# Lightning-AI/lit-llama

Hardware: NVIDIA H100
Metric: LLaMA-7B gptq.int4 decode tokens/sec (higher is better)
Workload: dtype bf16

## Files before the change

lit-llama_b200/csrc/api.cu:

```cuda
#include <algorithm>
#include <cstdlib>
#include <mutex>
#include <utility>
#include <vector>

#include "b2l_common.cuh"

namespace b2l {

extern void* g_attn_timeline;
int decode_step_persistent(const b2l_decode_args* d, b2l_stream_t stream);
int check_adapter_prefix(const b2l_adapter_prefix* pre, const char* who);
int check_lora(const b2l_lora* lo, int N, int K, const char* who);

static thread_local char g_err[512] = "";

void set_error(const char* fmt, ...) {
  va_list ap;
  va_start(ap, fmt);
  vsnprintf(g_err, sizeof(g_err), fmt, ap);
  va_end(ap);
}

int cuda_fail(cudaError_t e, const char* what) {
  set_error("%s: %s (%s)", what, cudaGetErrorString(e), cudaGetErrorName(e));
  (void)cudaGetLastError();
  return (int)e;
}

int sm_count() {
  static int n[B2L_MAX_DEVICES] = {};
  int dev = 0;
  if (cudaGetDevice(&dev) != cudaSuccess || dev < 0 || dev >= B2L_MAX_DEVICES) return 132;
  if (n[dev] == 0) {
    int v = 0;
    if (cudaDeviceGetAttribute(&v, cudaDevAttrMultiProcessorCount, dev) != cudaSuccess || v <= 0) v = 132;
    n[dev] = v;
  }
  return n[dev];
}

}

using namespace b2l;

extern "C" int b2l_version(void) { return 100; }

extern "C" const char* b2l_last_error(void) { return g_err; }

extern "C" int b2l_device_info(int* sm, int* cc_major, int* cc_minor) {
  int dev = 0;
  B2L_CUDA(cudaGetDevice(&dev));
  int a = 0, b = 0, c = 0;
  B2L_CUDA(cudaDeviceGetAttribute(&a, cudaDevAttrMultiProcessorCount, dev));
  B2L_CUDA(cudaDeviceGetAttribute(&b, cudaDevAttrComputeCapabilityMajor, dev));
  B2L_CUDA(cudaDeviceGetAttribute(&c, cudaDevAttrComputeCapabilityMinor, dev));
  if (sm) *sm = a;
  if (cc_major) *cc_major = b;
  if (cc_minor) *cc_minor = c;
  return 0;
}

struct PfWindow { const void* ptr[B2L_PF_SEGMENTS]; unsigned long long bytes[B2L_PF_SEGMENTS]; };

static size_t prefetch_distance() {
  static const long mb = [] { const char* e = getenv("B2L_PF_MB"); return e ? atol(e) : 0L; }();
  return mb > 0 ? (size_t)mb << 20 : 0;
}

static std::vector<PfWindow> prefetch_windows(const b2l_decode_args* d) {
  std::vector<std::pair<const uint8_t*, size_t>> ops;
  const bool w8 = (d->flags & B2L_F_W8) != 0;
  auto add = [&](const b2l_q4_weight& w) {
    ops.push_back({(const uint8_t*)w.qw_mma, w8 ? b2l_w8_tiled_i8_bytes(w.N, w.K) : b2l_q4_tiled_i8_bytes(w.N, w.K)});
  };
  for (int l = 0; l < d->n_layer; ++l) {
    add(d->layers[l].c_attn); add(d->layers[l].c_proj); add(d->layers[l].c_fc12); add(d->layers[l].mlp_proj);
  }
  add(d->lm_head);
  const size_t n = ops.size(), D = prefetch_distance();
  std::vector<PfWindow> out(n, PfWindow{});
  if (D == 0) return out;
  std::vector<size_t> start(n + 1, 0);
  for (size_t j = 0; j < n; ++j) start[j + 1] = start[j] + ops[j].second;
  for (size_t j = 0; j < n; ++j) {
    size_t lo = std::max(start[j] + D, start[j + 1]), hi = start[j + 1] + D;
    int sg = 0;
    size_t k = j + 1;
    size_t base = start[j + 1];
    while (lo < hi && sg < B2L_PF_SEGMENTS && k < j + 1 + n) {
      const auto& op = ops[k % n];
      const size_t op_lo = base, op_hi = base + op.second;
      if (lo < op_hi) {
        const size_t a = (lo - op_lo) & ~(size_t)127, b = std::min(hi, op_hi) - op_lo;
        if (b > a && op.first != nullptr) {
          out[j].ptr[sg] = op.first + a;
          out[j].bytes[sg] = (b - a + 15) & ~(size_t)15;
          ++sg;
        }
        lo = std::min(hi, op_hi);
      }
      base = op_hi;
      ++k;
    }
  }
  return out;
}

static int q4_call(const b2l_q4_weight& w, const void* x, int ldx, void* y, int ldy, int M, int sz_dtype, int prologue,
                   const void* norm_scale, float eps, int epilogue, const void* res, int ldres, int flags,
                   b2l_stream_t stream, void* trace = nullptr, void* batch_work = nullptr, const PfWindow* pf = nullptr,
                   const b2l_decode_args* kv_of = nullptr, int kv_layer = 0, const b2l_out_affine* aff = nullptr) {
  b2l_q4_linear_args a{};
  if (aff != nullptr) a.out_affine = *aff;
  if (kv_of != nullptr) {
    const int hs = kv_of->n_embd / kv_of->n_head;
    a.pf_kv[0] = kv_of->layers[kv_layer].k_cache; a.pf_kv[1] = kv_of->layers[kv_layer].v_cache;
    a.pf_rows = (const long long*)kv_of->input_pos;
    a.pf_rows_max = kv_of->S; a.pf_nseg = kv_of->B * kv_of->n_head; a.pf_row_bytes = hs * 2;
    a.pf_seg_stride = (unsigned long long)kv_of->S * hs * 2;
  }
  if (pf != nullptr)
    for (int i = 0; i < B2L_PF_SEGMENTS; ++i) { a.pf_ptr[i] = pf->ptr[i]; a.pf_bytes[i] = pf->bytes[i]; }
  a.x = x; a.ldx = ldx;
  const bool gemv = (M == 1 && w.qw_mma != nullptr);
  const bool batch = (!gemv && M <= 8 && w.qw_mma != nullptr && batch_work != nullptr);
  a.qw_tiled = (gemv || batch) ? w.qw_mma : w.qw_tiled; a.scales = w.scales; a.zeros = w.zeros; a.sz_dtype = sz_dtype;
  a.y = y; a.ldy = ldy;
  a.M = M; a.N = w.N; a.K = w.K;
  a.prologue = prologue; a.norm_scale = norm_scale; a.eps = eps;
  a.epilogue = epilogue; a.res = res; a.ldres = ldres;
  a.split_k = 0;
  a.flags = flags;
  a.trace = gemv ? trace : nullptr;
  if ((flags & B2L_F_Q4_BATCH_I8) && M > 1) {
    a.qw_tiled = w.qw_mma; a.trace = nullptr; a.workspace = batch_work;
    a.flags = flags & B2L_F_PDL;
    return b2l_q4_gemv_batch_i8(&a, stream);
  }
  if (flags & B2L_F_W8) {
    if (M > 1) {
      a.qw_tiled = w.qw_mma; a.trace = nullptr; a.workspace = batch_work;
      a.flags = flags & B2L_F_PDL;
      return b2l_w8_gemv_batch(&a, stream);
    }
    a.flags = flags & (B2L_F_PDL | B2L_F_DEBUG_NOCOMPUTE);
    return b2l_w8_gemv(&a, stream);
  }
  if (gemv) return b2l_q4_gemv(&a, stream);
  if (batch) {
    a.workspace = batch_work;
    return b2l_q4_gemv_batch(&a, stream);
  }
  if (a.qw_tiled == nullptr) {
    set_error("b2l_decode_step: weight has no tiling for batch %d", M);
    return B2L_E_STATE;
  }
  return b2l_q4_linear_tc(&a, stream);
}

static int q8_call(const b2l_decode_args* d, const b2l_q8_weight& w, const b2l_q8_weight* w2, const void* x, void* y,
                   const void* norm_scale, int epilogue, const void* res, const b2l_out_affine* aff, b2l_stream_t stream) {
  b2l_q8_linear_args a{};
  a.x = x; a.cb = w.cb; a.scb = w.scb;
  if (w2 != nullptr) { a.cb2 = w2->cb; a.scb2 = w2->scb; }
  a.y = y; a.N = w.N; a.K = w.K; a.threshold = d->q8_threshold;
  a.prologue = norm_scale != nullptr ? B2L_PRO_RMSNORM : B2L_PRO_NONE; a.norm_scale = norm_scale; a.eps = d->eps;
  a.epilogue = epilogue; a.res = res;
  if (aff != nullptr) a.out_affine = *aff;
  a.flags = d->flags & B2L_F_PDL;
  if (d->flags & B2L_F_Q8_BATCH)
    return b2l_q8_linear_batch(&a, d->B, d->batch_work, b2l_q8_linear_batch_workspace_bytes(w.K, d->B), stream);
  return b2l_q8_linear(&a, stream);
}

static int check_q8_weight(const b2l_q8_weight& w, int N, int K, const char* what, int l) {
// ... 85 lines not shown
  if (q8)
    if (int rc = check_q8(d)) return rc;
  if (d->flags & B2L_F_W8_BATCH) {
    B2L_CHECK_SUPPORTED(d->flags & B2L_F_W8, "b2l_decode_step: B2L_F_W8_BATCH needs B2L_F_W8 (gptq.int8)");
    B2L_CHECK_SUPPORTED(d->B >= 2 && d->B <= 16, "b2l_decode_step: B2L_F_W8_BATCH runs batches of 2..16, got B=%d", d->B);
    B2L_CHECK_SUPPORTED(d->plan == nullptr, "b2l_decode_step: B2L_F_W8_BATCH does not run in the persistent kernel (plan must be NULL)");
    B2L_CHECK_SUPPORTED(d->affines == nullptr && d->lm_head_affine.scale == nullptr && d->lm_head_affine.bias == nullptr,
                        "b2l_decode_step: B2L_F_W8_BATCH does not apply LLaMA-Adapter v2 affines (batch 1 only)");
    B2L_CHECK_ARG(d->batch_work != nullptr, "b2l_decode_step: B2L_F_W8_BATCH needs batch_work (b2l_w8_gemv_batch_workspace_bytes(max K, B) bytes)");
  } else if (d->flags & B2L_F_W8) {
    B2L_CHECK_SUPPORTED(d->B == 1, "b2l_decode_step: B2L_F_W8 (gptq.int8) runs batch 1 only, got B=%d", d->B);
    B2L_CHECK_SUPPORTED(d->plan == nullptr, "b2l_decode_step: B2L_F_W8 (gptq.int8) does not run in the persistent kernel (plan must be NULL)");
  }
  if (d->adapters != nullptr) {
    for (int l = 0; l < d->n_layer; ++l) {
      if (d->adapters[l].len == 0) continue;
      B2L_CHECK_SUPPORTED(d->plan == nullptr, "b2l_decode_step: adapters do not run in the persistent kernel (plan must be NULL)");
      if (int rc = check_adapter_prefix(&d->adapters[l], "b2l_decode_step")) return rc;
    }
  }
  if (d->loras != nullptr) {
    for (int l = 0; l < d->n_layer; ++l) {
      if (d->loras[l].r == 0) continue;
      B2L_CHECK_SUPPORTED(d->plan == nullptr, "b2l_decode_step: LoRA layers do not run in the persistent kernel (plan must be NULL)");
      if (int rc = check_lora(&d->loras[l], 3 * d->n_embd, d->n_embd, "b2l_decode_step")) return rc;
    }
  }
  const bool any_affine = d->affines != nullptr || d->lm_head_affine.scale != nullptr || d->lm_head_affine.bias != nullptr;
  if (any_affine) {
    B2L_CHECK_SUPPORTED(d->B == 1 || (d->flags & B2L_F_Q8_BATCH),
                        "b2l_decode_step: LLaMA-Adapter v2 affines run at batch 1 only, got B=%d", d->B);
    B2L_CHECK_SUPPORTED(d->plan == nullptr, "b2l_decode_step: LLaMA-Adapter v2 affines do not run in the persistent kernel (plan must be NULL)");
    B2L_CHECK_SUPPORTED(d->loras == nullptr, "b2l_decode_step: LLaMA-Adapter v2 affines and LoRA do not combine");
    auto ok = [](const b2l_out_affine& f) { return (f.scale == nullptr) == (f.bias == nullptr); };
    B2L_CHECK_ARG(ok(d->lm_head_affine), "b2l_decode_step: lm_head_affine needs both scale and bias (or neither)");
    B2L_CHECK_SUPPORTED(q8 || d->lm_head.qw_mma != nullptr, "b2l_decode_step: affines need the batch-1 tiling (qw_mma) of every weight");
    for (int l = 0; d->affines != nullptr && l < d->n_layer; ++l) {
      const b2l_layer_affine& f = d->affines[l];
      B2L_CHECK_ARG(ok(f.c_attn) && ok(f.c_proj) && ok(f.c_fc12) && ok(f.mlp_proj),
                    "b2l_decode_step: affines[%d] needs both scale and bias (or neither) per linear", l);
      const b2l_layer& L = d->layers[l];
      B2L_CHECK_SUPPORTED(q8 || (L.c_attn.qw_mma && L.c_proj.qw_mma && L.c_fc12.qw_mma && L.mlp_proj.qw_mma),
                          "b2l_decode_step: affines need the batch-1 tiling (qw_mma) of every weight");
    }
  }
  if (d->plan != nullptr) return decode_step_persistent(d, stream);
  const int C = d->n_embd, hs = C / d->n_head, B = d->B;
  const int fl = d->flags & ~(B2L_F_ROW_POS | B2L_F_STEPWISE);
  const int afl = d->flags & ~(B2L_F_W8 | B2L_F_Q8 | B2L_F_W8_BATCH | B2L_F_Q4_BATCH_I8 | B2L_F_Q8_BATCH);
  int rc;
  char* tlb = (char*)d->timeline;
  int li = 0;
  auto tl = [&]() -> void* { void* r = tlb ? (void*)(tlb + 512 * li) : nullptr; ++li; return r; };
  std::vector<PfWindow> pfw;
  if (B == 1 && d->lm_head.qw_mma != nullptr) pfw = prefetch_windows(d);
  static const int kv_prefetch = [] { const char* e = getenv("B2L_KV_PREFETCH"); return e ? atoi(e) : 0; }();
  const bool kv_ok = B == 1 && hs == 128 && d->lm_head.qw_mma != nullptr;
  int oi = 0;
  auto pf = [&]() -> const PfWindow* { const PfWindow* r = pfw.empty() ? nullptr : &pfw[oi]; ++oi; return r; };
  if ((rc = row_pos ? b2l_ring_advance_rows(d->input_pos, B, d->ring_start, d->S, stream)
                    : b2l_ring_advance(d->input_pos, stepwise ? B : 1, d->ring_start, d->S, stream)))
    return rc;
  const int aB = stepwise ? 1 : B, aT = stepwise ? B : 1;
  if ((rc = b2l_embedding(d->idx, d->idx_is_i64, d->wte, d->x, B, C, d->vocab, stream))) return rc;
  for (int l = 0; l < d->n_layer; ++l) {
    const b2l_layer& L = d->layers[l];
    const b2l_layer_affine* af = d->affines != nullptr ? &d->affines[l] : nullptr;
    const b2l_q8_layer* Q = q8 ? &d->q8_layers[l] : nullptr;
    void* t = tl();
    if ((rc = Q ? q8_call(d, Q->c_attn, nullptr, d->x, d->qkv, L.rms_1, B2L_EPI_STORE, nullptr, af ? &af->c_attn : nullptr, stream)
                : q4_call(L.c_attn, d->x, C, d->qkv, 3 * C, B, d->sz_dtype, B2L_PRO_RMSNORM, L.rms_1, d->eps, B2L_EPI_STORE,
                          nullptr, 0, fl, stream, t, d->batch_work, pf(), (kv_ok && kv_prefetch == 2) ? d : nullptr, l,
                          af ? &af->c_attn : nullptr)))
      return rc;
    if (d->loras != nullptr && d->loras[l].r != 0 &&
        (rc = b2l_lora_apply(&d->loras[l], d->x, C, L.rms_1, d->eps, d->qkv, 3 * C, B, 3 * C, C, fl & B2L_F_PDL, stream)))
      return rc;
    g_attn_timeline = tl();
    const b2l_adapter_prefix* pre = (d->adapters != nullptr && d->adapters[l].len != 0) ? &d->adapters[l] : nullptr;
    if ((rc = pre != nullptr
                  ? b2l_attention_adapter(d->qkv, L.k_cache, L.v_cache, d->rope, d->input_pos, d->ring_start, d->att,
                                          d->attn_work, aB, aT, d->n_head, hs, d->S, d->block_size, afl, pre, stream)
                  : b2l_attention(d->qkv, L.k_cache, L.v_cache, d->rope, d->input_pos, d->ring_start, d->att,
                                  d->attn_work, aB, aT, d->n_head, hs, d->S, d->block_size, afl, stream))) {
      g_attn_timeline = nullptr;
      return rc;
    }
    g_attn_timeline = nullptr;
    t = tl();
    if ((rc = Q ? q8_call(d, Q->c_proj, nullptr, d->att, d->x, nullptr, B2L_EPI_RESIDUAL, d->x, af ? &af->c_proj : nullptr, stream)
                : q4_call(L.c_proj, d->att, C, d->x, C, B, d->sz_dtype, B2L_PRO_NONE, nullptr, 0.f, B2L_EPI_RESIDUAL, d->x, C,
                          fl, stream, t, d->batch_work, pf(), nullptr, 0, af ? &af->c_proj : nullptr)))
      return rc;
    t = tl();
    if ((rc = Q ? q8_call(d, Q->c_fc1, &Q->c_fc2, d->x, d->hid, L.rms_2, B2L_EPI_SWIGLU, nullptr, af ? &af->c_fc12 : nullptr, stream)
                : q4_call(L.c_fc12, d->x, C, d->hid, d->n_hidden, B, d->sz_dtype, B2L_PRO_RMSNORM, L.rms_2, d->eps,
                          B2L_EPI_SWIGLU, nullptr, 0, fl, stream, t, d->batch_work, pf(), nullptr, 0, af ? &af->c_fc12 : nullptr)))
      return rc;
    const bool kvpf = kv_prefetch == 1 && kv_ok && l + 1 < d->n_layer;
    t = tl();
    if ((rc = Q ? q8_call(d, Q->mlp_proj, nullptr, d->hid, d->x, nullptr, B2L_EPI_RESIDUAL, d->x, af ? &af->mlp_proj : nullptr, stream)
                : q4_call(L.mlp_proj, d->hid, d->n_hidden, d->x, C, B, d->sz_dtype, B2L_PRO_NONE, nullptr, 0.f,
                          B2L_EPI_RESIDUAL, d->x, C, fl, stream, t, d->batch_work, pf(), kvpf ? d : nullptr, l + 1,
                          af ? &af->mlp_proj : nullptr)))
      return rc;
  }
  if (q8) return q8_call(d, d->q8_lm_head, nullptr, d->x, d->logits, d->ln_f, B2L_EPI_STORE, nullptr, &d->lm_head_affine, stream);
  return q4_call(d->lm_head, d->x, C, d->logits, d->vocab, B, d->sz_dtype, B2L_PRO_RMSNORM, d->ln_f, d->eps,
                 B2L_EPI_STORE, nullptr, 0, fl, stream, tl(), d->batch_work, pf(), nullptr, 0, &d->lm_head_affine);
}
```

lit-llama_b200/csrc/q4_gemv.cu:

```cuda
#include <cstdlib>

#include "q4_mma_common.cuh"

namespace b2l {
namespace q4mv {

struct Params {
  const __nv_bfloat16* x;
  const uint8_t* qwt;
  const void* scales; const void* zeros; int szdt;
  __nv_bfloat16* y;
  int N, K;
  int n_rb;
  int prologue; const __nv_bfloat16* norm_scale; float eps;
  int epilogue; const __nv_bfloat16* res;
  int nst;
  unsigned long long* tl;
  int nocompute;
  const uint8_t* pf_ptr[B2L_PF_SEGMENTS];
  uint32_t pf_bytes[B2L_PF_SEGMENTS];
  int pf_mode;
  const uint8_t* pf_kv[2]; const long long* pf_rows; int pf_rows_max, pf_nseg, pf_row_bytes; unsigned long long pf_seg_stride;
  int evict_first;
  const __nv_bfloat16* aff_scale; const __nv_bfloat16* aff_bias;
};

constexpr uint32_t PF_CHUNK = 16384;

__host__ __device__ inline uint32_t plane_stride(int K) { return (uint32_t)K + ((K % 128 == 0) ? 64u : 0u); }

struct SmemLayout {
  uint32_t ring, xf, zero, scratch, red, sxp, bars, total;
};
__host__ __device__ inline SmemLayout smem_layout(int nst, int K, int ndig) {
  SmemLayout L;
  uint32_t o = 0;
  L.ring = o;    o += (uint32_t)nst * STAGE_BYTES;
  L.xf = o;      o += (uint32_t)ndig * plane_stride(K);
  L.zero = o;    o += 16;
  L.scratch = o; o += 2 * NCW * MAX_HALVES * RB * 16;
  L.red = o;     o += 144;
  L.sxp = o;     o += NCW * 32 * 4;
  L.bars = o;    o += 2 * MAX_STAGES * 8;
  L.total = (o + 127u) & ~127u;
  return L;
}

__device__ __forceinline__ void l2_prefetch_bulk(const void* src, uint32_t bytes) {
  asm volatile("cp.async.bulk.prefetch.L2.global [%0], %1;" ::"l"(src), "r"(bytes) : "memory");
}
__device__ __forceinline__ void l2_prefetch_line(const void* src) {
  asm volatile("prefetch.global.L2 [%0];" ::"l"(src));
}
__device__ __forceinline__ void pf_slice(uint32_t bytes, uint32_t& lo, uint32_t& hi) {
  const uint32_t lines = (bytes + 127u) >> 7;
  lo = (uint32_t)(((unsigned long long)blockIdx.x * lines) / gridDim.x) << 7;
  hi = min((uint32_t)(((unsigned long long)(blockIdx.x + 1) * lines) / gridDim.x) << 7, bytes);
}
__device__ __forceinline__ void tma_bulk_g2s_hint(uint32_t dst, const void* src, uint32_t bytes, uint32_t mbar, uint64_t policy) {
  asm volatile(
      "cp.async.bulk.shared::cluster.global.mbarrier::complete_tx::bytes.L2::cache_hint [%0], [%1], %2, [%3], %4;" ::"r"(dst),
      "l"(src), "r"(bytes), "r"(mbar), "l"(policy)
      : "memory");
}

__device__ __forceinline__ uint32_t balanced_digits(int X) { return ((uint32_t)X + 0x00808080u) ^ 0x00808080u; }

template <bool W8> struct WTile {
  static constexpr int KB_BYTES = W8 ? 1024 : 512;
  static constexpr int KBP = HALF_STAGE_BYTES / KB_BYTES;
};

template <bool W8>
__device__ __forceinline__ void single_imma(int (&a)[2][4], const uint8_t* tile, const uint4& xb) {
  if constexpr (W8) {
    const uint4 w0 = *reinterpret_cast<const uint4*>(tile), w1 = *reinterpret_cast<const uint4*>(tile + 512);
    mma_u8s8_16832(a[0], w0.x, w0.y, w0.z, w0.w, xb.x, xb.y);
    mma_u8s8_16832(a[1], w1.x, w1.y, w1.z, w1.w, xb.z, xb.w);
  } else {
    const uint4 wv = *reinterpret_cast<const uint4*>(tile);
    mma_u8s8_16832(a[0], wv.x, wv.x & 0xf0f0f0f0u, wv.y, wv.y & 0xf0f0f0f0u, xb.x, xb.y);
    mma_u8s8_16832(a[1], wv.z, wv.z & 0xf0f0f0f0u, wv.w, wv.w & 0xf0f0f0f0u, xb.z, xb.w);
  }
}

template <int NH, bool W8>
__device__ __forceinline__ void kblock_imma(int (&acc)[MAX_HALVES][2][4], const uint8_t* wbase, const uint4& xb) {
#pragma unroll
  for (int h = 0; h < NH; ++h) single_imma<W8>(acc[h], wbase + h * HALF_STAGE_BYTES, xb);
}

template <int MAXC, int NDIG, bool W8, bool AFFINE>
__global__ void __launch_bounds__(NTHREADS, 2) q4_gemv_kernel(const Params p) {
  constexpr int KB_BYTES = WTile<W8>::KB_BYTES, KBP_PER_STAGE = WTile<W8>::KBP;
  extern __shared__ __align__(128) uint8_t smem[];
  const SmemLayout L = smem_layout(p.nst, p.K, NDIG);
  const uint32_t sbase = smem_u32(smem);
  const int tid = threadIdx.x, warp = tid >> 5, lane = tid & 31;
  const int n_kb = p.K / KB;
  const int spu2 = (n_kb + KBP_PER_STAGE - 1) / KBP_PER_STAGE, spu1 = (n_kb + 2 * KBP_PER_STAGE - 1) / (2 * KBP_PER_STAGE);
  const int rb_lo = (int)(((long long)blockIdx.x * p.n_rb) / gridDim.x);
  const int rb_hi = (int)(((long long)(blockIdx.x + 1) * p.n_rb) / gridDim.x);
  const int n_units = (rb_hi - rb_lo + 1) / 2;
  const int total_stages = ((rb_hi - rb_lo) / 2) * spu2 + ((rb_hi - rb_lo) & 1) * spu1;
  const uint32_t bar_full = sbase + L.bars, bar_empty = bar_full + MAX_STAGES * 8;
  const uint32_t PS = plane_stride(p.K);

  if (tid == 0) tl_min(p.tl, 0);
  if (tid == 0) {
    for (int i = 0; i < p.nst; ++i) {
      mbar_init(bar_full + i * 8, 1);
      mbar_init(bar_empty + i * 8, NCW);
    }
    asm volatile("fence.mbarrier_init.release.cluster;" ::: "memory");
  }
  if (tid < 4) reinterpret_cast<uint32_t*>(smem + L.zero)[tid] = 0u;
  __syncthreads();

  if (warp == PRODUCER_WARP) {
    if (lane == 0) {
      int slot = 0;
      uint32_t phase = 1;
      int it = 0;
      uint64_t policy = 0;
      if (p.evict_first) asm volatile("createpolicy.fractional.L2::evict_first.b64 %0, 1.0;" : "=l"(policy));
      for (int u = 0; u < n_units; ++u) {
        const int rb = rb_lo + 2 * u;
        const int halves = min(2, rb_hi - rb);
        const uint8_t* src = p.qwt + (size_t)rb * n_kb * KB_BYTES;
        const int per_stage = halves == 2 ? KBP_PER_STAGE : 2 * KBP_PER_STAGE;
        for (int kb0 = 0; kb0 < n_kb; kb0 += per_stage, ++it) {
          const int nkb = min(per_stage, n_kb - kb0);
          const uint32_t bytes = (uint32_t)nkb * KB_BYTES;
          mbar_wait(bar_empty + slot * 8, phase);
          mbar_expect_tx(bar_full + slot * 8, bytes * halves);
          for (int h = 0; h < halves; ++h) {
            const uint32_t dst = sbase + L.ring + slot * STAGE_BYTES + h * HALF_STAGE_BYTES;
            const uint8_t* from = src + ((size_t)h * n_kb + kb0) * KB_BYTES;
            if (p.evict_first) tma_bulk_g2s_hint(dst, from, bytes, bar_full + slot * 8, policy);
            else tma_bulk_g2s(dst, from, bytes, bar_full + slot * 8);
          }
          if (++slot == p.nst) { slot = 0; phase ^= 1; }
          if (it + 1 == min(total_stages, p.nst)) {
            pdl_launch_dependents();
            if (p.pf_mode == 1) {
#pragma unroll
              for (int sgi = 0; sgi < B2L_PF_SEGMENTS; ++sgi) {
                if (p.pf_bytes[sgi] == 0) continue;
                uint32_t lo, hi;
                pf_slice(p.pf_bytes[sgi], lo, hi);
#pragma unroll 1
                for (uint32_t o = lo; o < hi; o += PF_CHUNK) l2_prefetch_bulk(p.pf_ptr[sgi] + o, min(PF_CHUNK, hi - o));
              }
            }
          }
        }
      }
      if (total_stages == 0) pdl_launch_dependents();
      if (p.pf_kv[0] != nullptr) {
        long long rows = *p.pf_rows;
        rows = rows < 0 ? 0 : (rows > p.pf_rows_max ? p.pf_rows_max : rows);
        const uint32_t seg_bytes = (uint32_t)rows * (uint32_t)p.pf_row_bytes;
        const uint32_t cps = (seg_bytes + PF_CHUNK - 1) / PF_CHUNK;
        const uint32_t total = 2u * (uint32_t)p.pf_nseg * cps;
#pragma unroll 1
        for (uint32_t id = blockIdx.x; id < total; id += gridDim.x) {
          const uint32_t sg = id / cps, o = (id - sg * cps) * PF_CHUNK;
          const uint32_t which = sg >= (uint32_t)p.pf_nseg ? 1u : 0u;
          const uint8_t* base = p.pf_kv[which] + (size_t)(sg - which * p.pf_nseg) * p.pf_seg_stride;
          l2_prefetch_bulk(base + o, min(PF_CHUNK, seg_bytes - o));
        }
      }
    }
  } else if (warp < NCW) {
    float* red = reinterpret_cast<float*>(smem + L.red);
    int* red_sh = reinterpret_cast<int*>(smem + L.red + 128);
    {
      const bool norm = (p.prologue == B2L_PRO_RMSNORM);
      constexpr int NT = NCW * 32;
      constexpr uint32_t MAGIC_BITS = 0x4B400000u;
      uint4 xv[MAXC], gv[MAXC];
#pragma unroll
      for (int c = 0; c < MAXC; ++c) {
        const int k = (c * NT + tid) * 8;
        gv[c] = make_uint4(0, 0, 0, 0);
        if (norm && k < p.K) gv[c] = *reinterpret_cast<const uint4*>(p.norm_scale + k);
      }
      pdl_wait();
      if (tid == 0) tl_max(p.tl, 1);
#pragma unroll
      for (int c = 0; c < MAXC; ++c) {
        const int k = (c * NT + tid) * 8;
        xv[c] = make_uint4(0, 0, 0, 0);
        if (k < p.K) xv[c] = ld_coherent_u4(p.x + k);
      }
      const int nchunk = (p.K + NT * 8 - 1) / (NT * 8);
      float ss = 0.f;
      __nv_bfloat162 amax2 = __float2bfloat162_rn(0.f);
#pragma unroll
      for (int c = 0; c < MAXC; ++c) {
        if (c < nchunk) {
          const uint32_t w[4] = {xv[c].x, xv[c].y, xv[c].z, xv[c].w};
          const uint32_t g[4] = {gv[c].x, gv[c].y, gv[c].z, gv[c].w};
#pragma unroll
          for (int q = 0; q < 4; ++q) {
            const __nv_bfloat162 v = *reinterpret_cast<const __nv_bfloat162*>(&w[q]);
            if (norm) {
              amax2 = __hmax2(amax2, __habs2(__hmul2(v, *reinterpret_cast<const __nv_bfloat162*>(&g[q]))));
              const __nv_bfloat162 sq = __hmul2(v, v);
              const uint32_t su = *reinterpret_cast<const uint32_t*>(&sq);
              ss += __uint_as_float(su << 16) + __uint_as_float(su & 0xffff0000u);
            } else {
              amax2 = __hmax2(amax2, __habs2(v));
            }
          }
        }
      }
      float mx = fmaxf(__low2float(amax2), __high2float(amax2));
      ss = warp_sum(ss);
      mx = warp_max(mx);
      if (lane == 0) { red[warp] = ss; red[8 + warp] = mx; }
      named_bar_sync(1, NT);
      ss = 0.f; mx = 0.f;
#pragma unroll
      for (int w = 0; w < NCW; ++w) { ss += red[w]; mx = fmaxf(mx, red[8 + w]); }
// ... 89 lines not shown
              for (int i = 0; i < NPAIR; ++i) {
                const int kbl = i * NCW + warp;
                if (kbl < nkb) kblock_imma<MAX_HALVES, W8>(acc, st_base + kbl * KB_BYTES, *reinterpret_cast<const uint4*>(xq + kbl * xf_step));
              }
            }
          } else {
            if (nkb == 2 * KBP_PER_STAGE) {
#pragma unroll
              for (int i = 0; i < NSINGLE; ++i) {
                const int kbl = i * NCW + warp;
                single_imma<W8>(acc[i & 1], st_base + kbl * KB_BYTES, *reinterpret_cast<const uint4*>(xq + kbl * xf_step));
              }
            } else {
#pragma unroll
              for (int i = 0; i < NSINGLE; ++i) {
                const int kbl = i * NCW + warp;
                if (kbl < nkb) single_imma<W8>(acc[i & 1], st_base + kbl * KB_BYTES, *reinterpret_cast<const uint4*>(xq + kbl * xf_step));
              }
            }
          }
        }
        __syncwarp();
        if (lane == 0) mbar_arrive(bar_empty + slot * 8);
        if (++slot == p.nst) { slot = 0; phase ^= 1; }
      }
      const int buf = u & 1;
      named_bar_sync(4 + buf, NCW * 32 + 32);
      if (t4 < 2) {
        if (halves != MAX_HALVES) {
#pragma unroll
          for (int c = 0; c < 2; ++c)
#pragma unroll
            for (int i = 0; i < 4; ++i) acc[0][c][i] += acc[1][c][i];
        }
#pragma unroll
        for (int h = 0; h < MAX_HALVES; ++h) {
          const int c0 = acc[h][0][0] + acc[h][1][0], c1 = acc[h][0][1] + acc[h][1][1];
          const int c2 = acc[h][0][2] + acc[h][1][2], c3 = acc[h][0][3] + acc[h][1][3];
          int* dst = scratch + (((buf * NCW + warp) * MAX_HALVES + h) * RB + (lane >> 2)) * 4 + 2 * t4;
          if constexpr (W8) {
            *reinterpret_cast<int2*>(dst) = make_int2(c0, c1);
            *reinterpret_cast<int2*>(dst + 8 * 4) = make_int2(c2, c3);
          } else {
            *reinterpret_cast<int2*>(dst) = make_int2(c0 - c2, c1 - c3);
            *reinterpret_cast<int2*>(dst + 8 * 4) = make_int2(c2 >> 4, c3 >> 4);
          }
        }
      }
      __syncwarp();
      named_bar_arrive(6 + buf, NCW * 32 + 32);
    }
    if (tid == 0) tl_max(p.tl, 3);
  } else {
    if (p.pf_mode >= 2) {
      const uint32_t step = p.pf_mode == 2 ? 128u : 32u;
#pragma unroll
      for (int sgi = 0; sgi < B2L_PF_SEGMENTS; ++sgi) {
        if (p.pf_bytes[sgi] == 0) continue;
        uint32_t lo, hi;
        pf_slice(p.pf_bytes[sgi], lo, hi);
#pragma unroll 1
        for (uint32_t o = lo + lane * step; o < hi; o += 32 * step) l2_prefetch_line(p.pf_ptr[sgi] + o);
      }
    }
    float aff_s = 1.f, aff_b = 0.f;
    auto load_affine = [&](int u) {
      const int orow = (rb_lo + 2 * u + (lane >> 4)) * RB + (lane & 15);
      const int o = min(orow, p.N - 1);
      aff_s = bf2f(p.aff_scale[o]);
      aff_b = bf2f(p.aff_bias[o]);
    };
    if constexpr (AFFINE) {
      if (n_units > 0) load_affine(0);
    }
    pdl_wait();
    const int* red_sh = reinterpret_cast<const int*>(smem + L.red + 128);
    const int* scratch = reinterpret_cast<const int*>(smem + L.scratch);
    named_bar_sync(3, NCW * 32 + 32);
    long long sum_x = 0;
    {
      const int4* sp = reinterpret_cast<const int4*>(smem + L.sxp) + lane * 2;
      const int4 s0 = sp[0], s1 = sp[1];
      sum_x = (long long)s0.x + s0.y + s0.z + s0.w + s1.x + s1.y + s1.z + s1.w;
#pragma unroll
      for (int o = 16; o > 0; o >>= 1) sum_x += __shfl_xor_sync(0xffffffffu, sum_x, o);
    }
    const double dsum_x = (double)sum_x;
    const int sh = *red_sh;
    const double inv_scale = __longlong_as_double((long long)(1023 - sh) << 52);
    if (n_units > 0) named_bar_arrive(4, NCW * 32 + 32);
    if (n_units > 1) named_bar_arrive(5, NCW * 32 + 32);
    for (int u = 0; u < n_units; ++u) {
      const int rb = rb_lo + 2 * u;
      const int halves = min(2, rb_hi - rb);
      const int buf = u & 1;
      const int half = lane >> 4, row = lane & 15;
      const bool active = half < halves;
      const int orow = (rb + half) * RB + row;
      const int o = min(orow, p.N - 1);
      const float sc = load_sz(p.scales, p.szdt, o);
      const float zero = load_sz(p.zeros, p.szdt, o);
      if constexpr (AFFINE) {
        if (u > 0) load_affine(u);
      }
      float resv = 0.f;
      if (p.epilogue == B2L_EPI_RESIDUAL && active && orow < p.N) resv = bf2f(p.res[orow]);
      named_bar_sync(6 + buf, NCW * 32 + 32);
      int d0 = 0, d1 = 0, d2 = 0, d3 = 0;
#pragma unroll
      for (int w = 0; w < NCW; ++w) {
        const int4 v = *reinterpret_cast<const int4*>(scratch + (((buf * NCW + w) * MAX_HALVES + half) * RB + row) * 4);
        d0 += v.x; d1 += v.y; d2 += v.z; d3 += v.w;
      }
      if (u + 2 < n_units) named_bar_arrive(4 + buf, NCW * 32 + 32);
      const long long tq = (long long)d0 + ((long long)d1 << 8) + ((long long)d2 << 16) + ((long long)d3 << 24);
      const float tf = (float)(((double)tq - (double)zero * dsum_x) * inv_scale);
      float v = rbf(sc * tf);
// ... 92 lines not shown

using namespace b2l;
using namespace b2l::q4mv;

extern "C" size_t b2l_q4_tiled_i8_bytes(int N, int K) {
  if (N <= 0 || K <= 0 || K % KB != 0) return 0;
  return (size_t)((N + RB - 1) / RB) * (K / KB) * KB_BYTES;
}

extern "C" int b2l_q4_tile_i8(const void* qw, void* qw_tiled, int N, int K, b2l_stream_t stream) {
  B2L_CHECK_ARG(qw && qw_tiled && N > 0 && K > 0, "b2l_q4_tile_i8: bad argument");
  B2L_CHECK_SUPPORTED(K % KB == 0, "b2l_q4_tile_i8: in_features %d must be a multiple of %d", K, KB);
  const size_t total = b2l_q4_tiled_i8_bytes(N, K) / 4;
  q4_tile_i8_kernel<<<(unsigned)((total + 255) / 256), 256, 0, (cudaStream_t)stream>>>((const uint8_t*)qw, (uint32_t*)qw_tiled, N, K);
  B2L_LAUNCH_CHECK("q4_tile_i8_kernel");
  return 0;
}

extern "C" int b2l_q4_untile_i8(const void* qw_tiled, void* qw, int N, int K, b2l_stream_t stream) {
  B2L_CHECK_ARG(qw && qw_tiled && N > 0 && K > 0, "b2l_q4_untile_i8: bad argument");
  B2L_CHECK_SUPPORTED(K % KB == 0, "b2l_q4_untile_i8: in_features %d must be a multiple of %d", K, KB);
  const size_t total = (size_t)(K / 2) * N;
  q4_untile_i8_kernel<<<(unsigned)((total + 255) / 256), 256, 0, (cudaStream_t)stream>>>((const uint32_t*)qw_tiled, (uint8_t*)qw, N, K);
  B2L_LAUNCH_CHECK("q4_untile_i8_kernel");
  return 0;
}

extern "C" size_t b2l_w8_tiled_i8_bytes(int N, int K) {
  if (N <= 0 || K <= 0 || K % KB != 0) return 0;
  return (size_t)((N + RB - 1) / RB) * (K / KB) * WTile<true>::KB_BYTES;
}

extern "C" int b2l_w8_tile_i8(const void* qw, void* qw_tiled, int N, int K, b2l_stream_t stream) {
  B2L_CHECK_ARG(qw && qw_tiled && N > 0 && K > 0, "b2l_w8_tile_i8: bad argument");
  B2L_CHECK_SUPPORTED(K % KB == 0, "b2l_w8_tile_i8: in_features %d must be a multiple of %d", K, KB);
  const size_t total = b2l_w8_tiled_i8_bytes(N, K) / 4;
  w8_tile_i8_kernel<<<(unsigned)((total + 255) / 256), 256, 0, (cudaStream_t)stream>>>((const uint8_t*)qw, (uint32_t*)qw_tiled, N, K);
  B2L_LAUNCH_CHECK("w8_tile_i8_kernel");
  return 0;
}

extern "C" int b2l_w8_untile_i8(const void* qw_tiled, void* qw, int N, int K, b2l_stream_t stream) {
  B2L_CHECK_ARG(qw && qw_tiled && N > 0 && K > 0, "b2l_w8_untile_i8: bad argument");
  B2L_CHECK_SUPPORTED(K % KB == 0, "b2l_w8_untile_i8: in_features %d must be a multiple of %d", K, KB);
  const size_t total = (size_t)K * N;
  w8_untile_i8_kernel<<<(unsigned)((total + 255) / 256), 256, 0, (cudaStream_t)stream>>>((const uint8_t*)qw_tiled, (uint8_t*)qw, N, K);
  B2L_LAUNCH_CHECK("w8_untile_i8_kernel");
  return 0;
}

namespace {
constexpr int MAX_K = 12 * NCW * 32 * 8;

template <int MAXC, int NDIG, bool W8, bool AFFINE>
int launch_gemv_variant(const Params& p0, int ctas_per_sm, int grid_override, bool pdl, cudaStream_t stream) {
  Params p = p0;
  static const int env_kb = [] { const char* e = getenv("B2L_GEMV_SMEM_KB"); return e ? atoi(e) : 0; }();
  const uint32_t budget = (env_kb > 0 ? (uint32_t)env_kb : (ctas_per_sm >= 2 ? 110u : 224u)) * 1024u;
  const uint32_t fixed = smem_layout(0, p.K, NDIG).total;
  int nst = fixed + 2 * STAGE_BYTES <= budget ? (int)((budget - fixed) / STAGE_BYTES) : 0;
  if (nst > MAX_STAGES) nst = MAX_STAGES;
  static const int env_nst = [] { const char* e = getenv("B2L_GEMV_STAGES"); return e ? atoi(e) : 0; }();
  if (env_nst > 0 && nst > env_nst) nst = env_nst;
  if (nst < 2) {
    set_error("b2l_q4_gemv: K=%d does not leave room for the weight ring", p.K);
    return B2L_E_UNSUPPORTED;
  }
  p.nst = nst;
  const SmemLayout L = smem_layout(nst, p.K, NDIG);
  static DynSmemCache smem_cache;
  if (int rc = ensure_dyn_smem(q4_gemv_kernel<MAXC, NDIG, W8, AFFINE>, L.total, smem_cache)) return rc;
  int grid = grid_override > 0 ? grid_override : ctas_per_sm * sm_count();
  if (grid > p.n_rb) grid = p.n_rb;
  LaunchCfg lc(dim3(grid), dim3(NTHREADS), L.total, stream, pdl, 1);
  B2L_CUDA(cudaLaunchKernelEx(&lc.cfg, q4_gemv_kernel<MAXC, NDIG, W8, AFFINE>, p));
  return 0;
}

template <int MAXC, int NDIG, bool W8>
int launch_gemv(const Params& p, int ctas_per_sm, int grid_override, bool pdl, cudaStream_t stream) {
  if (p.aff_scale != nullptr) return launch_gemv_variant<MAXC, NDIG, W8, true>(p, ctas_per_sm, grid_override, pdl, stream);
  return launch_gemv_variant<MAXC, NDIG, W8, false>(p, ctas_per_sm, grid_override, pdl, stream);
}

template <bool W8>
int gemv_entry(const b2l_q4_linear_args* a, b2l_stream_t stream) {
  const char* fn = W8 ? "b2l_w8_gemv" : "b2l_q4_gemv";
  B2L_CHECK_ARG(a != nullptr, "%s: null args", fn);
  B2L_CHECK_ARG(a->x && a->qw_tiled && a->scales && a->zeros && a->y, "%s: null pointer", fn);
  B2L_CHECK_SUPPORTED(a->M == 1, "%s: M=%d (this kernel is the batch-1 path; use %s)", fn, a->M,
                      W8 ? "b2l_w8_gemm" : "b2l_q4_gemv_batch / b2l_q4_linear_tc");
  B2L_CHECK_SUPPORTED(a->K > 0 && a->K % KB == 0 && a->K <= MAX_K, "%s: K=%d must be a multiple of %d and <= %d", fn, a->K, KB, MAX_K);
  B2L_CHECK_ARG(a->N > 0, "%s: bad N", fn);
  B2L_CHECK_ARG(((uintptr_t)a->x % 16 == 0) && ((uintptr_t)a->qw_tiled % 16 == 0), "%s: x / qw_tiled must be 16-byte aligned", fn);
  B2L_CHECK_ARG(a->sz_dtype == B2L_BF16 || a->sz_dtype == B2L_F32, "%s: bad sz_dtype", fn);
  if (W8) B2L_CHECK_SUPPORTED((a->flags & ~(B2L_F_PDL | B2L_F_DEBUG_NOCOMPUTE)) == 0, "%s: unknown flags 0x%x", fn, a->flags);
  if (a->prologue == B2L_PRO_RMSNORM)
    B2L_CHECK_ARG(a->norm_scale && ((uintptr_t)a->norm_scale % 16 == 0), "%s: RMSNorm prologue needs a 16-byte aligned scale", fn);
  else
    B2L_CHECK_ARG(a->prologue == B2L_PRO_NONE, "%s: bad prologue %d", fn, a->prologue);
  if (a->epilogue == B2L_EPI_RESIDUAL) B2L_CHECK_ARG(a->res != nullptr, "%s: RESIDUAL epilogue needs res", fn);
  else if (a->epilogue == B2L_EPI_SWIGLU) B2L_CHECK_SUPPORTED(a->N % RB == 0, "%s: SWIGLU needs N %% 16 == 0", fn);
  else B2L_CHECK_ARG(a->epilogue == B2L_EPI_STORE, "%s: bad epilogue %d", fn, a->epilogue);
  B2L_CHECK_ARG((a->out_affine.scale == nullptr) == (a->out_affine.bias == nullptr),
                "%s: out_affine needs both scale and bias (or neither)", fn);

  Params p;
  p.aff_scale = (const __nv_bfloat16*)a->out_affine.scale;
  p.aff_bias = (const __nv_bfloat16*)a->out_affine.bias;
  p.x = (const __nv_bfloat16*)a->x;
  p.qwt = (const uint8_t*)a->qw_tiled;
  p.scales = a->scales; p.zeros = a->zeros; p.szdt = a->sz_dtype;
  p.y = (__nv_bfloat16*)a->y;
  p.N = a->N; p.K = a->K;
  p.n_rb = (a->N + RB - 1) / RB;
  p.prologue = a->prologue; p.norm_scale = (const __nv_bfloat16*)a->norm_scale; p.eps = a->eps;
  p.epilogue = a->epilogue; p.res = (const __nv_bfloat16*)a->res;
  p.nst = 0;
  p.tl = (unsigned long long*)a->trace;
  p.nocompute = (a->flags & B2L_F_DEBUG_NOCOMPUTE) ? 1 : 0;
  static const int env_pf_mode = [] { const char* e = getenv("B2L_PF_MODE"); return e ? atoi(e) : 1; }();
  static const int env_evict = [] { const char* e = getenv("B2L_PF_EVICT"); return e ? atoi(e) : 0; }();
  p.pf_mode = 0;
  p.evict_first = env_evict;
  p.pf_kv[0] = p.pf_kv[1] = nullptr; p.pf_rows = nullptr; p.pf_rows_max = p.pf_nseg = p.pf_row_bytes = 0; p.pf_seg_stride = 0;
  if (a->pf_kv[0] != nullptr) {
    B2L_CHECK_ARG(a->pf_kv[1] != nullptr && a->pf_rows != nullptr && a->pf_rows_max > 0 && a->pf_nseg > 0 && a->pf_row_bytes > 0 &&
                      a->pf_row_bytes % 16 == 0 && a->pf_seg_stride % 16 == 0 && ((uintptr_t)a->pf_kv[0] % 16 == 0) &&
                      ((uintptr_t)a->pf_kv[1] % 16 == 0) && (unsigned long long)a->pf_rows_max * a->pf_row_bytes < (1ull << 31),
                  "%s: bad strided prefetch hint", fn);
    p.pf_kv[0] = (const uint8_t*)a->pf_kv[0]; p.pf_kv[1] = (const uint8_t*)a->pf_kv[1];
    p.pf_rows = a->pf_rows; p.pf_rows_max = a->pf_rows_max; p.pf_nseg = a->pf_nseg; p.pf_row_bytes = a->pf_row_bytes;
    p.pf_seg_stride = a->pf_seg_stride;
  }
  for (int i = 0; i < B2L_PF_SEGMENTS; ++i) {
    p.pf_ptr[i] = (const uint8_t*)a->pf_ptr[i];
    p.pf_bytes[i] = 0;
    if (a->pf_ptr[i] != nullptr && a->pf_bytes[i] != 0) {
      B2L_CHECK_ARG(((uintptr_t)a->pf_ptr[i] % 16 == 0) && (a->pf_bytes[i] % 16 == 0) && a->pf_bytes[i] < (1ull << 31),
                    "%s: prefetch segment %d must be 16-byte aligned, a multiple of 16 and < 2 GiB", fn, i);
      p.pf_bytes[i] = (uint32_t)a->pf_bytes[i];
      p.pf_mode = env_pf_mode;
    }
  }
  static const int env_cps = [] { const char* e = getenv("B2L_GEMV_CTAS_PER_SM"); return e ? atoi(e) : 0; }();
  const bool pdl = (a->flags & B2L_F_PDL) != 0;
  cudaStream_t st = (cudaStream_t)stream;
  const int grid = a->split_k;
  if (a->K <= 12288) return launch_gemv<6, 3, W8>(p, env_cps > 0 ? env_cps : 2, grid, pdl, st);
  if (a->K <= 16384) return launch_gemv<12, 3, W8>(p, env_cps > 0 ? env_cps : 2, grid, pdl, st);
  return launch_gemv<12, 3, W8>(p, 1, grid, pdl, st);
}
}

extern "C" int b2l_q4_gemv(const b2l_q4_linear_args* a, b2l_stream_t stream) { return gemv_entry<false>(a, stream); }

extern "C" int b2l_w8_gemv(const b2l_q4_linear_args* a, b2l_stream_t stream) { return gemv_entry<true>(a, stream); }
```

Before: 596.3.

## Drop L2 prefetch machinery and pick one CTA per SM when the ring holds all stages

```diff
diff --git a/lit-llama_b200/csrc/api.cu b/lit-llama_b200/csrc/api.cu
--- a/lit-llama_b200/csrc/api.cu
+++ b/lit-llama_b200/csrc/api.cu
@@ -1,8 +1,4 @@
-#include <algorithm>
-#include <cstdlib>
 #include <mutex>
-#include <utility>
-#include <vector>
 
 #include "b2l_common.cuh"
 
@@ -61,67 +57,11 @@
   return 0;
 }
 
-struct PfWindow { const void* ptr[B2L_PF_SEGMENTS]; unsigned long long bytes[B2L_PF_SEGMENTS]; };
-
-static size_t prefetch_distance() {
-  static const long mb = [] { const char* e = getenv("B2L_PF_MB"); return e ? atol(e) : 0L; }();
-  return mb > 0 ? (size_t)mb << 20 : 0;
-}
-
-static std::vector<PfWindow> prefetch_windows(const b2l_decode_args* d) {
-  std::vector<std::pair<const uint8_t*, size_t>> ops;
-  const bool w8 = (d->flags & B2L_F_W8) != 0;
-  auto add = [&](const b2l_q4_weight& w) {
-    ops.push_back({(const uint8_t*)w.qw_mma, w8 ? b2l_w8_tiled_i8_bytes(w.N, w.K) : b2l_q4_tiled_i8_bytes(w.N, w.K)});
-  };
-  for (int l = 0; l < d->n_layer; ++l) {
-    add(d->layers[l].c_attn); add(d->layers[l].c_proj); add(d->layers[l].c_fc12); add(d->layers[l].mlp_proj);
-  }
-  add(d->lm_head);
-  const size_t n = ops.size(), D = prefetch_distance();
-  std::vector<PfWindow> out(n, PfWindow{});
-  if (D == 0) return out;
-  std::vector<size_t> start(n + 1, 0);
-  for (size_t j = 0; j < n; ++j) start[j + 1] = start[j] + ops[j].second;
-  for (size_t j = 0; j < n; ++j) {
-    size_t lo = std::max(start[j] + D, start[j + 1]), hi = start[j + 1] + D;
-    int sg = 0;
-    size_t k = j + 1;
-    size_t base = start[j + 1];
-    while (lo < hi && sg < B2L_PF_SEGMENTS && k < j + 1 + n) {
-      const auto& op = ops[k % n];
-      const size_t op_lo = base, op_hi = base + op.second;
-      if (lo < op_hi) {
-        const size_t a = (lo - op_lo) & ~(size_t)127, b = std::min(hi, op_hi) - op_lo;
-        if (b > a && op.first != nullptr) {
-          out[j].ptr[sg] = op.first + a;
-          out[j].bytes[sg] = (b - a + 15) & ~(size_t)15;
-          ++sg;
-        }
-        lo = std::min(hi, op_hi);
-      }
-      base = op_hi;
-      ++k;
-    }
-  }
-  return out;
-}
-
 static int q4_call(const b2l_q4_weight& w, const void* x, int ldx, void* y, int ldy, int M, int sz_dtype, int prologue,
                    const void* norm_scale, float eps, int epilogue, const void* res, int ldres, int flags,
-                   b2l_stream_t stream, void* trace = nullptr, void* batch_work = nullptr, const PfWindow* pf = nullptr,
-                   const b2l_decode_args* kv_of = nullptr, int kv_layer = 0, const b2l_out_affine* aff = nullptr) {
+                   b2l_stream_t stream, void* trace = nullptr, void* batch_work = nullptr, const b2l_out_affine* aff = nullptr) {
   b2l_q4_linear_args a{};
   if (aff != nullptr) a.out_affine = *aff;
-  if (kv_of != nullptr) {
-    const int hs = kv_of->n_embd / kv_of->n_head;
-    a.pf_kv[0] = kv_of->layers[kv_layer].k_cache; a.pf_kv[1] = kv_of->layers[kv_layer].v_cache;
-    a.pf_rows = (const long long*)kv_of->input_pos;
-    a.pf_rows_max = kv_of->S; a.pf_nseg = kv_of->B * kv_of->n_head; a.pf_row_bytes = hs * 2;
-    a.pf_seg_stride = (unsigned long long)kv_of->S * hs * 2;
-  }
-  if (pf != nullptr)
-    for (int i = 0; i < B2L_PF_SEGMENTS; ++i) { a.pf_ptr[i] = pf->ptr[i]; a.pf_bytes[i] = pf->bytes[i]; }
   a.x = x; a.ldx = ldx;
   const bool gemv = (M == 1 && w.qw_mma != nullptr);
   const bool batch = (!gemv && M <= 8 && w.qw_mma != nullptr && batch_work != nullptr);
@@ -313,12 +253,6 @@
   char* tlb = (char*)d->timeline;
   int li = 0;
   auto tl = [&]() -> void* { void* r = tlb ? (void*)(tlb + 512 * li) : nullptr; ++li; return r; };
-  std::vector<PfWindow> pfw;
-  if (B == 1 && d->lm_head.qw_mma != nullptr) pfw = prefetch_windows(d);
-  static const int kv_prefetch = [] { const char* e = getenv("B2L_KV_PREFETCH"); return e ? atoi(e) : 0; }();
-  const bool kv_ok = B == 1 && hs == 128 && d->lm_head.qw_mma != nullptr;
-  int oi = 0;
-  auto pf = [&]() -> const PfWindow* { const PfWindow* r = pfw.empty() ? nullptr : &pfw[oi]; ++oi; return r; };
   if ((rc = row_pos ? b2l_ring_advance_rows(d->input_pos, B, d->ring_start, d->S, stream)
                     : b2l_ring_advance(d->input_pos, stepwise ? B : 1, d->ring_start, d->S, stream)))
     return rc;
@@ -331,8 +265,7 @@
     void* t = tl();
     if ((rc = Q ? q8_call(d, Q->c_attn, nullptr, d->x, d->qkv, L.rms_1, B2L_EPI_STORE, nullptr, af ? &af->c_attn : nullptr, stream)
                 : q4_call(L.c_attn, d->x, C, d->qkv, 3 * C, B, d->sz_dtype, B2L_PRO_RMSNORM, L.rms_1, d->eps, B2L_EPI_STORE,
-                          nullptr, 0, fl, stream, t, d->batch_work, pf(), (kv_ok && kv_prefetch == 2) ? d : nullptr, l,
-                          af ? &af->c_attn : nullptr)))
+                          nullptr, 0, fl, stream, t, d->batch_work, af ? &af->c_attn : nullptr)))
       return rc;
     if (d->loras != nullptr && d->loras[l].r != 0 &&
         (rc = b2l_lora_apply(&d->loras[l], d->x, C, L.rms_1, d->eps, d->qkv, 3 * C, B, 3 * C, C, fl & B2L_F_PDL, stream)))
@@ -351,22 +284,20 @@
     t = tl();
     if ((rc = Q ? q8_call(d, Q->c_proj, nullptr, d->att, d->x, nullptr, B2L_EPI_RESIDUAL, d->x, af ? &af->c_proj : nullptr, stream)
                 : q4_call(L.c_proj, d->att, C, d->x, C, B, d->sz_dtype, B2L_PRO_NONE, nullptr, 0.f, B2L_EPI_RESIDUAL, d->x, C,
-                          fl, stream, t, d->batch_work, pf(), nullptr, 0, af ? &af->c_proj : nullptr)))
+                          fl, stream, t, d->batch_work, af ? &af->c_proj : nullptr)))
       return rc;
     t = tl();
     if ((rc = Q ? q8_call(d, Q->c_fc1, &Q->c_fc2, d->x, d->hid, L.rms_2, B2L_EPI_SWIGLU, nullptr, af ? &af->c_fc12 : nullptr, stream)
                 : q4_call(L.c_fc12, d->x, C, d->hid, d->n_hidden, B, d->sz_dtype, B2L_PRO_RMSNORM, L.rms_2, d->eps,
-                          B2L_EPI_SWIGLU, nullptr, 0, fl, stream, t, d->batch_work, pf(), nullptr, 0, af ? &af->c_fc12 : nullptr)))
-      return rc;
-    const bool kvpf = kv_prefetch == 1 && kv_ok && l + 1 < d->n_layer;
+                          B2L_EPI_SWIGLU, nullptr, 0, fl, stream, t, d->batch_work, af ? &af->c_fc12 : nullptr)))
+      return rc;
     t = tl();
     if ((rc = Q ? q8_call(d, Q->mlp_proj, nullptr, d->hid, d->x, nullptr, B2L_EPI_RESIDUAL, d->x, af ? &af->mlp_proj : nullptr, stream)
                 : q4_call(L.mlp_proj, d->hid, d->n_hidden, d->x, C, B, d->sz_dtype, B2L_PRO_NONE, nullptr, 0.f,
-                          B2L_EPI_RESIDUAL, d->x, C, fl, stream, t, d->batch_work, pf(), kvpf ? d : nullptr, l + 1,
-                          af ? &af->mlp_proj : nullptr)))
+                          B2L_EPI_RESIDUAL, d->x, C, fl, stream, t, d->batch_work, af ? &af->mlp_proj : nullptr)))
       return rc;
   }
   if (q8) return q8_call(d, d->q8_lm_head, nullptr, d->x, d->logits, d->ln_f, B2L_EPI_STORE, nullptr, &d->lm_head_affine, stream);
   return q4_call(d->lm_head, d->x, C, d->logits, d->vocab, B, d->sz_dtype, B2L_PRO_RMSNORM, d->ln_f, d->eps,
-                 B2L_EPI_STORE, nullptr, 0, fl, stream, tl(), d->batch_work, pf(), nullptr, 0, &d->lm_head_affine);
-}
+                 B2L_EPI_STORE, nullptr, 0, fl, stream, tl(), d->batch_work, &d->lm_head_affine);
+}
diff --git a/lit-llama_b200/csrc/q4_gemv.cu b/lit-llama_b200/csrc/q4_gemv.cu
--- a/lit-llama_b200/csrc/q4_gemv.cu
+++ b/lit-llama_b200/csrc/q4_gemv.cu
@@ -1,4 +1,4 @@
-#include <cstdlib>
+#include <algorithm>
 
 #include "q4_mma_common.cuh"
 
@@ -17,15 +17,8 @@
   int nst;
   unsigned long long* tl;
   int nocompute;
-  const uint8_t* pf_ptr[B2L_PF_SEGMENTS];
-  uint32_t pf_bytes[B2L_PF_SEGMENTS];
-  int pf_mode;
-  const uint8_t* pf_kv[2]; const long long* pf_rows; int pf_rows_max, pf_nseg, pf_row_bytes; unsigned long long pf_seg_stride;
-  int evict_first;
   const __nv_bfloat16* aff_scale; const __nv_bfloat16* aff_bias;
 };
-
-constexpr uint32_t PF_CHUNK = 16384;
 
 __host__ __device__ inline uint32_t plane_stride(int K) { return (uint32_t)K + ((K % 128 == 0) ? 64u : 0u); }
 
@@ -46,24 +39,6 @@
   return L;
 }
 
-__device__ __forceinline__ void l2_prefetch_bulk(const void* src, uint32_t bytes) {
-  asm volatile("cp.async.bulk.prefetch.L2.global [%0], %1;" ::"l"(src), "r"(bytes) : "memory");
-}
-__device__ __forceinline__ void l2_prefetch_line(const void* src) {
-  asm volatile("prefetch.global.L2 [%0];" ::"l"(src));
-}
-__device__ __forceinline__ void pf_slice(uint32_t bytes, uint32_t& lo, uint32_t& hi) {
-  const uint32_t lines = (bytes + 127u) >> 7;
-  lo = (uint32_t)(((unsigned long long)blockIdx.x * lines) / gridDim.x) << 7;
-  hi = min((uint32_t)(((unsigned long long)(blockIdx.x + 1) * lines) / gridDim.x) << 7, bytes);
-}
-__device__ __forceinline__ void tma_bulk_g2s_hint(uint32_t dst, const void* src, uint32_t bytes, uint32_t mbar, uint64_t policy) {
-  asm volatile(
-      "cp.async.bulk.shared::cluster.global.mbarrier::complete_tx::bytes.L2::cache_hint [%0], [%1], %2, [%3], %4;" ::"r"(dst),
-      "l"(src), "r"(bytes), "r"(mbar), "l"(policy)
-      : "memory");
-}
-
 __device__ __forceinline__ uint32_t balanced_digits(int X) { return ((uint32_t)X + 0x00808080u) ^ 0x00808080u; }
 
 template <bool W8> struct WTile {
@@ -122,8 +97,6 @@
       int slot = 0;
       uint32_t phase = 1;
       int it = 0;
-      uint64_t policy = 0;
-      if (p.evict_first) asm volatile("createpolicy.fractional.L2::evict_first.b64 %0, 1.0;" : "=l"(policy));
       for (int u = 0; u < n_units; ++u) {
         const int rb = rb_lo + 2 * u;
         const int halves = min(2, rb_hi - rb);
@@ -137,40 +110,13 @@
           for (int h = 0; h < halves; ++h) {
             const uint32_t dst = sbase + L.ring + slot * STAGE_BYTES + h * HALF_STAGE_BYTES;
             const uint8_t* from = src + ((size_t)h * n_kb + kb0) * KB_BYTES;
-            if (p.evict_first) tma_bulk_g2s_hint(dst, from, bytes, bar_full + slot * 8, policy);
-            else tma_bulk_g2s(dst, from, bytes, bar_full + slot * 8);
+            tma_bulk_g2s(dst, from, bytes, bar_full + slot * 8);
           }
           if (++slot == p.nst) { slot = 0; phase ^= 1; }
-          if (it + 1 == min(total_stages, p.nst)) {
-            pdl_launch_dependents();
-            if (p.pf_mode == 1) {
-#pragma unroll
-              for (int sgi = 0; sgi < B2L_PF_SEGMENTS; ++sgi) {
-                if (p.pf_bytes[sgi] == 0) continue;
-                uint32_t lo, hi;
-                pf_slice(p.pf_bytes[sgi], lo, hi);
-#pragma unroll 1
-                for (uint32_t o = lo; o < hi; o += PF_CHUNK) l2_prefetch_bulk(p.pf_ptr[sgi] + o, min(PF_CHUNK, hi - o));
-              }
-            }
-          }
+          if (it + 1 == min(total_stages, p.nst)) pdl_launch_dependents();
         }
       }
       if (total_stages == 0) pdl_launch_dependents();
-      if (p.pf_kv[0] != nullptr) {
-        long long rows = *p.pf_rows;
-        rows = rows < 0 ? 0 : (rows > p.pf_rows_max ? p.pf_rows_max : rows);
-        const uint32_t seg_bytes = (uint32_t)rows * (uint32_t)p.pf_row_bytes;
-        const uint32_t cps = (seg_bytes + PF_CHUNK - 1) / PF_CHUNK;
-        const uint32_t total = 2u * (uint32_t)p.pf_nseg * cps;
-#pragma unroll 1
-        for (uint32_t id = blockIdx.x; id < total; id += gridDim.x) {
-          const uint32_t sg = id / cps, o = (id - sg * cps) * PF_CHUNK;
-          const uint32_t which = sg >= (uint32_t)p.pf_nseg ? 1u : 0u;
-          const uint8_t* base = p.pf_kv[which] + (size_t)(sg - which * p.pf_nseg) * p.pf_seg_stride;
-          l2_prefetch_bulk(base + o, min(PF_CHUNK, seg_bytes - o));
-        }
-      }
     }
   } else if (warp < NCW) {
     float* red = reinterpret_cast<float*>(smem + L.red);
@@ -366,17 +312,6 @@
     }
     if (tid == 0) tl_max(p.tl, 3);
   } else {
-    if (p.pf_mode >= 2) {
-      const uint32_t step = p.pf_mode == 2 ? 128u : 32u;
-#pragma unroll
-      for (int sgi = 0; sgi < B2L_PF_SEGMENTS; ++sgi) {
-        if (p.pf_bytes[sgi] == 0) continue;
-        uint32_t lo, hi;
-        pf_slice(p.pf_bytes[sgi], lo, hi);
-#pragma unroll 1
-        for (uint32_t o = lo + lane * step; o < hi; o += 32 * step) l2_prefetch_line(p.pf_ptr[sgi] + o);
-      }
-    }
     float aff_s = 1.f, aff_b = 0.f;
     auto load_affine = [&](int u) {
       const int orow = (rb_lo + 2 * u + (lane >> 4)) * RB + (lane & 15);
@@ -575,16 +510,33 @@
 namespace {
 constexpr int MAX_K = 12 * NCW * 32 * 8;
 
+template <int NDIG>
+int ring_stages(int K, uint32_t budget) {
+  const uint32_t fixed = smem_layout(0, K, NDIG).total;
+  const int nst = fixed + 2 * STAGE_BYTES <= budget ? (int)((budget - fixed) / STAGE_BYTES) : 0;
+  return nst > MAX_STAGES ? MAX_STAGES : nst;
+}
+
+template <bool W8>
+int cta_stages(int rbs, int n_kb) {
+  constexpr int KBP = WTile<W8>::KBP;
+  return (rbs / 2) * ((n_kb + KBP - 1) / KBP) + (rbs & 1) * ((n_kb + 2 * KBP - 1) / (2 * KBP));
+}
+
 template <int MAXC, int NDIG, bool W8, bool AFFINE>
-int launch_gemv_variant(const Params& p0, int ctas_per_sm, int grid_override, bool pdl, cudaStream_t stream) {
+int launch_gemv_variant(const Params& p0, int grid_override, bool pdl, cudaStream_t stream) {
   Params p = p0;
-  static const int env_kb = [] { const char* e = getenv("B2L_GEMV_SMEM_KB"); return e ? atoi(e) : 0; }();
-  const uint32_t budget = (env_kb > 0 ? (uint32_t)env_kb : (ctas_per_sm >= 2 ? 110u : 224u)) * 1024u;
-  const uint32_t fixed = smem_layout(0, p.K, NDIG).total;
-  int nst = fixed + 2 * STAGE_BYTES <= budget ? (int)((budget - fixed) / STAGE_BYTES) : 0;
-  if (nst > MAX_STAGES) nst = MAX_STAGES;
-  static const int env_nst = [] { const char* e = getenv("B2L_GEMV_STAGES"); return e ? atoi(e) : 0; }();
-  if (env_nst > 0 && nst > env_nst) nst = env_nst;
+  int ctas_per_sm = p.K <= 16384 ? 2 : 1;
+  int nst = ring_stages<NDIG>(p.K, (ctas_per_sm == 2 ? 110u : 224u) * 1024u);
+  if (ctas_per_sm == 2) {
+    const int sms = sm_count(), n_kb = p.K / KB;
+    const int one = ring_stages<NDIG>(p.K, 113u * 1024u);
+    const int rb_max = (p.n_rb + sms - 1) / sms, rb_min = p.n_rb / sms;
+    if (std::max(cta_stages<W8>(rb_max, n_kb), cta_stages<W8>(rb_min, n_kb)) <= one) {
+      ctas_per_sm = 1;
+      nst = one;
+    }
+  }
   if (nst < 2) {
     set_error("b2l_q4_gemv: K=%d does not leave room for the weight ring", p.K);
     return B2L_E_UNSUPPORTED;
@@ -601,9 +553,9 @@
 }
 
 template <int MAXC, int NDIG, bool W8>
-int launch_gemv(const Params& p, int ctas_per_sm, int grid_override, bool pdl, cudaStream_t stream) {
-  if (p.aff_scale != nullptr) return launch_gemv_variant<MAXC, NDIG, W8, true>(p, ctas_per_sm, grid_override, pdl, stream);
-  return launch_gemv_variant<MAXC, NDIG, W8, false>(p, ctas_per_sm, grid_override, pdl, stream);
+int launch_gemv(const Params& p, int grid_override, bool pdl, cudaStream_t stream) {
+  if (p.aff_scale != nullptr) return launch_gemv_variant<MAXC, NDIG, W8, true>(p, grid_override, pdl, stream);
+  return launch_gemv_variant<MAXC, NDIG, W8, false>(p, grid_override, pdl, stream);
 }
 
 template <bool W8>
@@ -642,37 +594,11 @@
   p.nst = 0;
   p.tl = (unsigned long long*)a->trace;
   p.nocompute = (a->flags & B2L_F_DEBUG_NOCOMPUTE) ? 1 : 0;
-  static const int env_pf_mode = [] { const char* e = getenv("B2L_PF_MODE"); return e ? atoi(e) : 1; }();
-  static const int env_evict = [] { const char* e = getenv("B2L_PF_EVICT"); return e ? atoi(e) : 0; }();
-  p.pf_mode = 0;
-  p.evict_first = env_evict;
-  p.pf_kv[0] = p.pf_kv[1] = nullptr; p.pf_rows = nullptr; p.pf_rows_max = p.pf_nseg = p.pf_row_bytes = 0; p.pf_seg_stride = 0;
-  if (a->pf_kv[0] != nullptr) {
-    B2L_CHECK_ARG(a->pf_kv[1] != nullptr && a->pf_rows != nullptr && a->pf_rows_max > 0 && a->pf_nseg > 0 && a->pf_row_bytes > 0 &&
-                      a->pf_row_bytes % 16 == 0 && a->pf_seg_stride % 16 == 0 && ((uintptr_t)a->pf_kv[0] % 16 == 0) &&
-                      ((uintptr_t)a->pf_kv[1] % 16 == 0) && (unsigned long long)a->pf_rows_max * a->pf_row_bytes < (1ull << 31),
-                  "%s: bad strided prefetch hint", fn);
-    p.pf_kv[0] = (const uint8_t*)a->pf_kv[0]; p.pf_kv[1] = (const uint8_t*)a->pf_kv[1];
-    p.pf_rows = a->pf_rows; p.pf_rows_max = a->pf_rows_max; p.pf_nseg = a->pf_nseg; p.pf_row_bytes = a->pf_row_bytes;
-    p.pf_seg_stride = a->pf_seg_stride;
-  }
-  for (int i = 0; i < B2L_PF_SEGMENTS; ++i) {
-    p.pf_ptr[i] = (const uint8_t*)a->pf_ptr[i];
-    p.pf_bytes[i] = 0;
-    if (a->pf_ptr[i] != nullptr && a->pf_bytes[i] != 0) {
-      B2L_CHECK_ARG(((uintptr_t)a->pf_ptr[i] % 16 == 0) && (a->pf_bytes[i] % 16 == 0) && a->pf_bytes[i] < (1ull << 31),
-                    "%s: prefetch segment %d must be 16-byte aligned, a multiple of 16 and < 2 GiB", fn, i);
-      p.pf_bytes[i] = (uint32_t)a->pf_bytes[i];
-      p.pf_mode = env_pf_mode;
-    }
-  }
-  static const int env_cps = [] { const char* e = getenv("B2L_GEMV_CTAS_PER_SM"); return e ? atoi(e) : 0; }();
   const bool pdl = (a->flags & B2L_F_PDL) != 0;
   cudaStream_t st = (cudaStream_t)stream;
   const int grid = a->split_k;
-  if (a->K <= 12288) return launch_gemv<6, 3, W8>(p, env_cps > 0 ? env_cps : 2, grid, pdl, st);
-  if (a->K <= 16384) return launch_gemv<12, 3, W8>(p, env_cps > 0 ? env_cps : 2, grid, pdl, st);
-  return launch_gemv<12, 3, W8>(p, 1, grid, pdl, st);
+  if (a->K <= 12288) return launch_gemv<6, 3, W8>(p, grid, pdl, st);
+  return launch_gemv<12, 3, W8>(p, grid, pdl, st);
 }
 }
 
```

After: 616.2 (median of 6 runs). 1.03x the previous value.
